# ucla-mobility/QuantV2X

Measured on AMD Instinct MI355X. Metric: frames/sec/node (N-agent int8 BEV fusion), higher is better.
Workload: dtype i8

## Files before the change

quantv2x_amd/csrc/common.h:

```cpp
#pragma once
#include <hip/hip_runtime.h>
#include <stdint.h>

#include "../../include/qv2x.h"

namespace qv2x {

int fail(int code, const char* fmt, ...);
int hip_check(hipError_t e, const char* what);

typedef int v4i __attribute__((ext_vector_type(4)));
typedef int v16i __attribute__((ext_vector_type(16)));
typedef float v4f __attribute__((ext_vector_type(4)));
typedef float v16f __attribute__((ext_vector_type(16)));

__device__ __forceinline__ float q_code(float y, float delta, float zp) {
    const float rdelta = 1.0f / delta;
    const float t = y * rdelta;
    float k = rintf(t);
    const bool doubtful = (fabsf(t - k) > 0.4997f) & (fabsf(t) < 1100.0f);
    if (__builtin_amdgcn_ballot_w64(doubtful) != 0) k = rintf(y / delta);
    float c = k + zp;
    c = fmaxf(c, 0.0f);
    return fminf(c, 255.0f);
}

__device__ __forceinline__ void q_add(float y, int e, float rdelta, float zp, float low, unsigned& c) {
    float t = __builtin_fmaf(y, rdelta, zp);
    t = fmaxf(t, low);
    c = __builtin_amdgcn_cvt_pk_u8_f32(t, e, c);
}
__device__ __forceinline__ int q_pack4(float y0, float y1, float y2, float y3, float delta, float rdelta, float zp, float lowc = 8388608.0f) {
    (void)delta;
    const float low = lowc - 8388608.0f;
    unsigned c = 0;
    q_add(y0, 0, rdelta, zp, low, c);
    q_add(y1, 1, rdelta, zp, low, c);
    q_add(y2, 2, rdelta, zp, low, c);
    q_add(y3, 3, rdelta, zp, low, c);
    return (int)(c ^ 0x80808080u);
}
__device__ __forceinline__ float q_code_mul(float y, float delta, float zp) {
    const float rdelta = 1.0f / delta;
    return fminf(fmaxf(rintf(__builtin_fmaf(y, rdelta, zp)), 0.0f), 255.0f);
}

__device__ __forceinline__ void q_sandwich_add(float y, int e, float rdelta, float za, float zb, unsigned& ca, unsigned& cb) {
    ca = __builtin_amdgcn_cvt_pk_u8_f32(__builtin_fmaf(y, rdelta, za), e, ca);
    cb = __builtin_amdgcn_cvt_pk_u8_f32(__builtin_fmaf(y, rdelta, zb), e, cb);
}
__device__ __forceinline__ int q_sandwich_finish(unsigned ca, unsigned cb, float y0, float y1, float y2, float y3, float delta, float zp, float low) {
    if ((__builtin_amdgcn_ballot_w64(ca != cb) != 0) | (low > 0.0f)) {
        const float y[4] = {y0, y1, y2, y3};
        ca = 0;
#pragma unroll
        for (int e = 0; e < 4; ++e) ca = __builtin_amdgcn_cvt_pk_u8_f32(fmaxf(rintf(y[e] / delta) + zp, low), e, ca);
    }
    return (int)(ca ^ 0x80808080u);
}
__device__ __forceinline__ int q_pack4_div(float y0, float y1, float y2, float y3, float delta, float rdelta, float zp, float lowc = 8388608.0f) {
    const float za = zp + 1.0e-4f, zb = zp - 1.0e-4f;
    unsigned ca = 0, cb = 0;
    q_sandwich_add(y0, 0, rdelta, za, zb, ca, cb);
    q_sandwich_add(y1, 1, rdelta, za, zb, ca, cb);
    q_sandwich_add(y2, 2, rdelta, za, zb, ca, cb);
    q_sandwich_add(y3, 3, rdelta, za, zb, ca, cb);
    return q_sandwich_finish(ca, cb, y0, y1, y2, y3, delta, zp, lowc - 8388608.0f);
}

__device__ __forceinline__ int mfma32_row(int r, int lane) { return (r & 3) + 8 * (r >> 2) + 4 * (lane >> 5); }

}
```

quantv2x_amd/csrc/heads_f32.hip:

```cpp
#include "fuse_att.h"

namespace qv2x {

enum { ROWS_GLOBAL = 0, ROWS_DECODE = 2, ROWS_FUSE = 3 };

#ifdef QV2X_HEADS_TRACE
__device__ long long g_heads_trace[32768 * 6];
#define HTRACE(k) do { const int hb_ = ((blockIdx.x >> 3) & 1) * (gridDim.x >> 1) + (blockIdx.x >> 4) * 8 + (blockIdx.x & 7); if (threadIdx.x == 0 && hb_ < 32768) g_heads_trace[hb_ * 6 + (k)] = __builtin_amdgcn_s_memtime(); } while (0)
#else
#define HTRACE(k) do { } while (0)
#endif

struct HeadArgs {
    const float* x; int R, hw, cout, cout_pad;
    const float* w; const float* bias; const float* da; const float* za; float* out;
};

template <int SRC, int NA = 1, bool U8 = false>
__device__ __forceinline__ void rows_heads_tile(const HeadArgs& h, const FuseArgs& fa, const int tm, float* smem, const SceneList* sl = nullptr) {
    float* rows = smem;
    HTRACE(0);
    const int lane = threadIdx.x & 63, wave = __builtin_amdgcn_readfirstlane(threadIdx.x >> 6);
    const int nct = h.cout_pad >> 5;
    const int par = lane >> 5;
// ... 152 lines not shown
            for (int hf = 0; hf < 2; ++hf)
#pragma unroll
                for (int r2 = 0; r2 < 4; ++r2) {
                    float y = c16[hf][r2];
                    if (d > 0.0f) y = U8 ? q_code(y, d, z) : (q_code(y, d, z) - z) * d;
                    tr[16 * hf + 4 * (lane >> 4) + r2][lane & 15] = y;
                }
        } else {
            const int co = ct * 32 + (lane & 31);
            const float d = h.da[co], z = h.za[co];
#pragma unroll
            for (int r2 = 0; r2 < 16; ++r2) {
                float y = acc[r2];
                if (d > 0.0f) y = U8 ? q_code(y, d, z) : (q_code(y, d, z) - z) * d;
                tr[mfma32_row(r2, lane)][lane & 31] = y;
            }
        }
        __builtin_amdgcn_s_waitcnt(0xc07f);
        __builtin_amdgcn_wave_barrier();
        const int mm = tm * 32 + (lane & 31);
        const int bi = mm / h.hw, cell = mm - bi * h.hw;
        float* ob = h.out + (size_t)bi * h.cout * h.hw + cell;
        uint8_t* ob8 = (uint8_t*)h.out + (size_t)bi * h.cout * h.hw + cell;
#pragma unroll
        for (int c = 0; c < 16; ++c) {
            const int ch = ct * 32 + par + 2 * c;
            if (ch < h.cout && mm < h.R) {
                if (U8) ob8[(size_t)ch * h.hw] = (uint8_t)tr[lane & 31][par + 2 * c];
                else ob[(size_t)ch * h.hw] = tr[lane & 31][par + 2 * c];
            }
        }
    }
    HTRACE(4);
}

template <int SRC, bool U8 = false>
__global__ __launch_bounds__(256) void rows_heads_kernel(const HeadArgs h, const FuseArgs fa) {
    __shared__ __attribute__((aligned(16))) float smem[32 * 256];
    rows_heads_tile<SRC, 1, U8>(h, fa, blockIdx.x, smem);
}

template <int NA, bool U8 = false>
__global__ __launch_bounds__(256) void fuse_heads_kernel(const HeadArgs h, const FuseArgs fa, const SceneList sl) {
    __shared__ __attribute__((aligned(16))) float smem[32 * 256];
    rows_heads_tile<ROWS_FUSE, NA, U8>(h, fa, blockIdx.x, smem, &sl);
}

__global__ __launch_bounds__(256) void rows_heads_pair_kernel(const HeadArgs h0, const HeadArgs h1, const FuseArgs fa1) {
    __shared__ __attribute__((aligned(16))) float smem[32 * 256];
    const int tile = (blockIdx.x >> 4) * 8 + (blockIdx.x & 7);
    if (((blockIdx.x >> 3) & 1) == 0) {
        if (tile * 32 < h0.R) rows_heads_tile<ROWS_GLOBAL>(h0, fa1, tile, smem);
    } else {
        if (tile * 32 < h1.R) rows_heads_tile<ROWS_DECODE>(h1, fa1, tile, smem);
    }
}

static int head_args(const char* who, int R, int hw, int cout, int cout_pad, const float* w, const float* bias, const float* da,
                     const float* za, float* out, HeadArgs& h) {
    if (!w || !bias || !da || !za || !out) return fail(QV2X_EINVAL, "%s: null pointer", who);
    if (R <= 0 || hw <= 0 || R % hw || cout <= 0 || cout > cout_pad || cout_pad % 32 || cout_pad > 96)
        return fail(QV2X_EINVAL, "%s: R=%d hw=%d cout=%d cout_pad=%d (cout_pad in {32, 64, 96})", who, R, hw, cout, cout_pad);
    if ((uintptr_t)w & 15) return fail(QV2X_EALIGN, "%s: w must be 16-byte aligned", who);
    h.x = nullptr; h.R = R; h.hw = hw; h.cout = cout; h.cout_pad = cout_pad; h.w = w; h.bias = bias; h.da = da; h.za = za; h.out = out;
    return QV2X_OK;
}

static int wire_check(const char* who, int wire, int cout, const float* da_host) {
    if (wire != QV2X_WIRE_F32 && wire != QV2X_WIRE_U8) return fail(QV2X_EINVAL, "%s: wire %d (QV2X_WIRE_F32 or QV2X_WIRE_U8)", who, wire);
    if (wire == QV2X_WIRE_U8) {
        if (!da_host) return fail(QV2X_EINVAL, "%s: the u8 wire needs da_host (the host copy of da)", who);
        for (int c = 0; c < cout; ++c)
            if (!(da_host[c] > 0.0f)) return fail(QV2X_EINVAL, "%s: the u8 wire needs an output quantizer on every channel (da[%d] = %g)", who, c, da_host[c]);
    }
    return QV2X_OK;
}

template <bool U8>
__global__ __launch_bounds__(256) void assemble_bands_kernel(const uint8_t* __restrict__ slabs, long long slab_bytes, int world, int planes, int cout,
                                                             int h, int w, const float* __restrict__ da, const float* __restrict__ za,
                                                             float* __restrict__ out) {
    const int r = blockIdx.y / planes, p = blockIdx.y - r * planes;
    const int y0 = (int)((long long)r * h / world), y1 = (int)((long long)(r + 1) * h / world);
    const int n = (y1 - y0) * w;
    if (n == 0) return;
    const size_t so = (size_t)p * n;
    const uint8_t* s8 = slabs + (size_t)r * slab_bytes + so;
    const float* s32 = (const float*)(slabs + (size_t)r * slab_bytes) + so;
    const size_t dof = (size_t)p * h * w + (size_t)y0 * w;
    float* dst = out + dof;
    float d = 1.0f, z = 0.0f;
    if (U8) { const int c = p % cout; d = da[c]; z = za[c]; }
    auto one = [&](int i) __attribute__((always_inline)) { return U8 ? ((float)s8[i] - z) * d : s32[i]; };
    int head = (int)((4 - (dof & 3)) & 3);
    if (head > n || ((so + head) & 3)) head = n;
    const int nv = (n - head) >> 2;
    const int tid = blockIdx.x * 256 + threadIdx.x, nt = gridDim.x * 256;
    for (int i = tid; i < head; i += nt) dst[i] = one(i);
    for (int v = tid; v < nv; v += nt) {
        const int i = head + 4 * v;
        float4 o;
        if (U8) {
            const unsigned cw = *(const unsigned*)(s8 + i);
            o = make_float4(((float)(cw & 0xff) - z) * d, ((float)((cw >> 8) & 0xff) - z) * d, ((float)((cw >> 16) & 0xff) - z) * d, ((float)(cw >> 24) - z) * d);
        } else {
            o = *(const float4*)(s32 + i);
        }
        *(float4*)(dst + i) = o;
    }
    for (int i = head + 4 * nv + tid; i < n; i += nt) dst[i] = one(i);
}

__global__ __launch_bounds__(256) void decode_lut_kernel(const uint8_t* __restrict__ codes, int R, int levels, int kc,
                                                         const float4* __restrict__ lut, const float4* __restrict__ bias,
                                                         float4* __restrict__ out) {
    const int lane = threadIdx.x & 63;
    int r = blockIdx.x * 4 + (threadIdx.x >> 6);
    r = __builtin_amdgcn_readfirstlane(r);
    if (r >= R) return;
    float4 v = bias[lane];
    for (int l = 0; l < levels; ++l) {
        const float4 t = lut[((size_t)l * kc + codes[(size_t)l * R + r]) * 64 + lane];
        v.x += t.x; v.y += t.y; v.z += t.z; v.w += t.w;
    }
    out[(size_t)r * 64 + lane] = v;
}

__global__ __launch_bounds__(256) void single_heads_lut_kernel(const uint8_t* __restrict__ codes, int R, int hw, int levels, int kc, int cout,
                                                               int groups, const float* __restrict__ tables, const float* __restrict__ bias,
                                                               const float* __restrict__ da, const float* __restrict__ za, float* __restrict__ out) {
    extern __shared__ __attribute__((aligned(16))) float tab[];
    const int nt = levels * kc * cout;
    for (int i = threadIdx.x; i < nt; i += blockDim.x) tab[i] = tables[i];
    for (int i = threadIdx.x; i < cout; i += blockDim.x) { tab[nt + i] = bias[i]; tab[nt + cout + i] = da[i]; tab[nt + 2 * cout + i] = za[i]; }
    __syncthreads();
    const int lane = threadIdx.x & 63, wv = threadIdx.x >> 6;
    for (int g = 0; g < groups; ++g) {
        const int m = (blockIdx.x * groups + g) * 64 + lane;
        if (m >= R) break;
        const int agent = m / hw, cell = m - agent * hw;
        const float* row[4];
        for (int l = 0; l < levels; ++l) row[l] = tab + ((size_t)l * kc + codes[(size_t)l * R + m]) * cout;
        float* ob = out + (size_t)agent * cout * hw + cell;
        for (int c = wv; c < cout; c += 4) {
            float y = tab[nt + c];
            for (int l = 0; l < levels; ++l) y += row[l][c];
            const float d = tab[nt + cout + c], z = tab[nt + 2 * cout + c];
            if (d > 0.0f) y = (q_code(y, d, z) - z) * d;
            ob[(size_t)c * hw] = y;
        }
    }
}

__global__ __launch_bounds__(1024, 1) void table_heads_kernel(const uint8_t* __restrict__ codes, int R, int hw, int levels, int kc, int CT, int ST, int c0, int c1,
                                                             const float* __restrict__ tables, const float* __restrict__ bias, const float* __restrict__ da,
                                                             const float* __restrict__ za, float* __restrict__ out0, float* __restrict__ out1) {
    extern __shared__ __attribute__((aligned(16))) float tab[];
    const int CT4 = (CT + 3) & ~3, rows = levels * kc;
    float* cst = tab + (size_t)rows * ST;
    for (int i = threadIdx.x; i < rows * (ST / 4); i += blockDim.x) {
        const int row = i / (ST / 4), q = i - row * (ST / 4);
        v4f v = {0.f, 0.f, 0.f, 0.f};
#pragma unroll
        for (int e = 0; e < 4; ++e)
            if (4 * q + e < CT) v[e] = tables[(size_t)row * CT + 4 * q + e];
        *(v4f*)(tab + (size_t)row * ST + 4 * q) = v;
    }
    for (int i = threadIdx.x; i < CT4; i += blockDim.x) {
        cst[i] = i < CT ? bias[i] : 0.f; cst[CT4 + i] = i < CT ? da[i] : -1.f; cst[2 * CT4 + i] = i < CT ? za[i] : 0.f;
    }
    __syncthreads();
    const int lane = threadIdx.x & 63, wave = threadIdx.x >> 6, nw = blockDim.x >> 6;
    const int runs = (R + 63) / 64;
    for (int run = blockIdx.x * nw + wave; run < runs; run += gridDim.x * nw) {
        const int m = run * 64 + lane;
        const int mc = m < R ? m : R - 1;
        const int agent = mc / hw, cell = mc - agent * hw;
        const float* rp[4];
#pragma unroll
        for (int l = 0; l < 4; ++l) rp[l] = tab + (size_t)(l < levels ? l * kc + codes[(size_t)l * R + mc] : 0) * ST;
        float* o0 = out0 ? out0 + (size_t)agent * c0 * hw + cell : nullptr;
        float* o1 = out1 ? out1 + (size_t)agent * c1 * hw + cell : nullptr;
        for (int g = 0; g < CT4 / 4; ++g) {
            v4f y = *(const v4f*)(cst + 4 * g);
            const v4f d4 = *(const v4f*)(cst + CT4 + 4 * g), z4 = *(const v4f*)(cst + 2 * CT4 + 4 * g);
#pragma unroll
            for (int l = 0; l < 4; ++l)
                if (l < levels) { const v4f t = *(const v4f*)(rp[l] + 4 * g); y[0] += t[0]; y[1] += t[1]; y[2] += t[2]; y[3] += t[3]; }
#pragma unroll
            for (int e = 0; e < 4; ++e) {
                const int c = 4 * g + e;
                float v = y[e];
                if (d4[e] > 0.0f) v = (q_code(v, d4[e], z4[e]) - z4[e]) * d4[e];
                if (m < R && c < CT) {
                    if (c < c0) { if (o0) o0[(size_t)c * hw] = v; }
                    else if (o1) o1[(size_t)(c - c0) * hw] = v;
                }
            }
        }
    }
}

__global__ __launch_bounds__(256) void dequant_i8_kernel(const int8_t* __restrict__ in, int n, int h, int w, int c, int ax, float delta,
                                                         float* __restrict__ out) {
    const size_t total = (size_t)n * h * w * (c / 4);
    for (size_t i = (size_t)blockIdx.x * blockDim.x + threadIdx.x; i < total; i += (size_t)gridDim.x * blockDim.x) {
        const int c4 = (int)(i % (c / 4));
        const size_t pix = i / (c / 4);
        const int x = (int)(pix % w), y = (int)((pix / w) % h), img = (int)(pix / ((size_t)w * h));
        const char4 v = *(const char4*)(in + (((size_t)img * (h + 2) + y + 1) * (w + 2) + x + 1) * c + c4 * 4);
        *(float4*)(out + pix * c + c4 * 4) = make_float4((float)((int)v.x + ax) * delta, (float)((int)v.y + ax) * delta,
                                                         (float)((int)v.z + ax) * delta, (float)((int)v.w + ax) * delta);
    }
}

}

extern "C" int qv2x_dequant_i8_f32(const int8_t* in, int n, int h, int w, int c, int zp, float delta, float* out, void* stream) {
    using namespace qv2x;
    if (!in || !out) return fail(QV2X_EINVAL, "qv2x_dequant_i8_f32: null pointer");
    if (n <= 0 || h <= 0 || w <= 0 || c <= 0 || c % 4) return fail(QV2X_EINVAL, "qv2x_dequant_i8_f32: bad shape (c %% 4 == 0)");
    const size_t total = (size_t)n * h * w * (c / 4);
    const int blocks = (int)((total + 255) / 256 < 4096 ? (total + 255) / 256 : 4096);
    dequant_i8_kernel<<<blocks, 256, 0, (hipStream_t)stream>>>(in, n, h, w, c, 128 - zp, delta, out);
    return hip_check(hipGetLastError(), "qv2x_dequant_i8_f32 launch");
}

extern "C" int qv2x_heads_f32(const float* x, int R, int hw, int cout, int cout_pad, const float* w, const float* bias,
                              const float* da, const float* za, float* out, void* stream) {
    using namespace qv2x;
    HeadArgs h;
    if (!x) return fail(QV2X_EINVAL, "qv2x_heads_f32: null pointer");
    if (int rc = head_args("qv2x_heads_f32", R, hw, cout, cout_pad, w, bias, da, za, out, h)) return rc;
    if ((uintptr_t)x & 15) return fail(QV2X_EALIGN, "qv2x_heads_f32: x must be 16-byte aligned");
    h.x = x;
    rows_heads_kernel<ROWS_GLOBAL><<<(R + 31) / 32, 256, 0, (hipStream_t)stream>>>(h, FuseArgs{});
    return hip_check(hipGetLastError(), "qv2x_heads_f32 launch");
}

namespace qv2x {
static int fuse_heads_launch(const char* who, const qv2x_fuse_desc* d, int n_scenes, const int64_t* scene_offset, const int32_t* scene_agents,
                             const uint8_t* codes, const float* lut, const float* lut_bias, const float* feats, const double* pairwise,
                             const long long* range, int cout, int cout_pad, const float* w, const float* bias, const float* da, const float* za,
                             bool u8, void* out, float* fused_tap, void* stream) {
    if (!scene_offset || !scene_agents || !d) return fail(QV2X_EINVAL, "%s: null pointer", who);
    if (n_scenes < 1 || n_scenes > MAX_SCENES) return fail(QV2X_EINVAL, "%s: 1..%d scenes, got %d", who, MAX_SCENES, n_scenes);
    SceneList sl{};
    int most = 1;
    for (int s = 0; s < n_scenes; ++s) {
        if (scene_offset[s] < 0 || (feats && scene_offset[s] % 4) || scene_agents[s] < 1 || scene_agents[s] > MAXA || scene_agents[s] > d->max_cav || d->ego >= scene_agents[s])
            return fail(QV2X_EINVAL, "%s: scene %d: offset %lld, agents %d (1..%d, <= max_cav, > ego)", who, s, (long long)scene_offset[s], scene_agents[s], MAXA);
        sl.off[s] = scene_offset[s]; sl.agents[s] = scene_agents[s];
        most = scene_agents[s] > most ? scene_agents[s] : most;
    }
    qv2x_fuse_desc d1 = *d;
    d1.agents = most;
    FuseArgs a;
    if (int rc = fuse_args_from_desc(&d1, codes, lut, lut_bias, feats, pairwise, who, a)) return rc;
    if (range) {
        if (int rc = fuse_band_range(who, range[0], range[1], a)) return rc;
        if (!out) return fail(QV2X_EINVAL, "%s: null pointer", who);
        if (a.n_cells == 0) return QV2X_OK;
    }
    a.fused = (float4*)fused_tap;
    HeadArgs h;
    if (int rc = head_args(who, n_scenes * a.n_cells, a.n_cells, cout, cout_pad, w, bias, da, za, (float*)out, h)) return rc;
    const dim3 grid((h.R + 31) / 32);
    hipStream_t st = (hipStream_t)stream;
    if (u8) {
        switch (fuse_bound(most)) {
            case 1: fuse_heads_kernel<1, true><<<grid, 256, 0, st>>>(h, a, sl); break;
            case 2: fuse_heads_kernel<2, true><<<grid, 256, 0, st>>>(h, a, sl); break;
            case 4: fuse_heads_kernel<4, true><<<grid, 256, 0, st>>>(h, a, sl); break;
            default: fuse_heads_kernel<MAXA, true><<<grid, 256, 0, st>>>(h, a, sl); break;
        }
        return hip_check(hipGetLastError(), who);
    }
    switch (fuse_bound(most)) {
        case 1: fuse_heads_kernel<1><<<grid, 256, 0, st>>>(h, a, sl); break;
        case 2: fuse_heads_kernel<2><<<grid, 256, 0, st>>>(h, a, sl); break;
        case 4: fuse_heads_kernel<4><<<grid, 256, 0, st>>>(h, a, sl); break;
        default: fuse_heads_kernel<MAXA><<<grid, 256, 0, st>>>(h, a, sl); break;
    }
    return hip_check(hipGetLastError(), who);
}
}

extern "C" int qv2x_fuse_heads_batch_f32(const qv2x_fuse_desc* d, int n_scenes, const int64_t* scene_offset, const int32_t* scene_agents,
                                         const uint8_t* codes, const float* lut, const float* lut_bias, const float* feats, const double* pairwise,
                                         int cout, int cout_pad, const float* w, const float* bias, const float* da, const float* za,
                                         float* out, float* fused_tap, void* stream) {
    return qv2x::fuse_heads_launch("qv2x_fuse_heads_batch_f32", d, n_scenes, scene_offset, scene_agents, codes, lut, lut_bias, feats, pairwise, nullptr,
                                   cout, cout_pad, w, bias, da, za, false, out, fused_tap, stream);
}

extern "C" int qv2x_fuse_heads_band(const qv2x_fuse_desc* d, int n_scenes, const int64_t* scene_offset, const int32_t* scene_agents,
                                    const uint8_t* codes, const float* lut, const float* lut_bias, const float* feats, const double* pairwise,
                                    int64_t cell0, int64_t n_cells, int cout, int cout_pad, const float* w, const float* bias, const float* da,
                                    const float* za, int wire, const float* da_host, void* out, float* fused_tap, void* stream) {
    using namespace qv2x;
    if (int rc = wire_check("qv2x_fuse_heads_band", wire, cout, da_host)) return rc;
    const long long range[2] = {(long long)cell0, (long long)n_cells};
    return fuse_heads_launch("qv2x_fuse_heads_band", d, n_scenes, scene_offset, scene_agents, codes, lut, lut_bias, feats, pairwise, range,
                             cout, cout_pad, w, bias, da, za, wire == QV2X_WIRE_U8, out, fused_tap, stream);
}

extern "C" int qv2x_heads_band(const float* x, int n_scenes, int64_t n_cells, int cout, int cout_pad, const float* w, const float* bias,
                               const float* da, const float* za, int wire, const float* da_host, void* out, void* stream) {
    using namespace qv2x;
    const char* who = "qv2x_heads_band";
    if (int rc = wire_check(who, wire, cout, da_host)) return rc;
    if (!x || !out) return fail(QV2X_EINVAL, "%s: null pointer", who);
    if (n_scenes < 1 || n_cells < 0 || n_cells * n_scenes > 0x7fffffffLL) return fail(QV2X_EINVAL, "%s: %d scenes of %lld cells", who, n_scenes, (long long)n_cells);
    if (n_cells == 0) return QV2X_OK;
    HeadArgs h;
    if (int rc = head_args(who, (int)(n_scenes * n_cells), (int)n_cells, cout, cout_pad, w, bias, da, za, (float*)out, h)) return rc;
    if ((uintptr_t)x & 15) return fail(QV2X_EALIGN, "%s: x must be 16-byte aligned", who);
    h.x = x;
    if (wire == QV2X_WIRE_U8) rows_heads_kernel<ROWS_GLOBAL, true><<<(h.R + 31) / 32, 256, 0, (hipStream_t)stream>>>(h, FuseArgs{});
    else rows_heads_kernel<ROWS_GLOBAL><<<(h.R + 31) / 32, 256, 0, (hipStream_t)stream>>>(h, FuseArgs{});
    return hip_check(hipGetLastError(), who);
}

extern "C" int qv2x_assemble_bands(const uint8_t* slabs, int world, int64_t slab_bytes, int frames, int cout, int h, int w, int wire,
                                   const float* da, const float* za, float* out, void* stream) {
    using namespace qv2x;
    const char* who = "qv2x_assemble_bands";
    if (!slabs || !out) return fail(QV2X_EINVAL, "%s: null pointer", who);
    if (wire != QV2X_WIRE_F32 && wire != QV2X_WIRE_U8) return fail(QV2X_EINVAL, "%s: wire %d (QV2X_WIRE_F32 or QV2X_WIRE_U8)", who, wire);
    if (wire == QV2X_WIRE_U8 && (!da || !za)) return fail(QV2X_EINVAL, "%s: the u8 wire needs da and za", who);
    if (world < 1 || frames < 1 || cout < 1 || h < 1 || w < 1 || (long long)h * w > 0x7fffffffLL || (long long)world * frames * cout > 65535)
        return fail(QV2X_EINVAL, "%s: world=%d frames=%d cout=%d h=%d w=%d (world * frames * cout <= 65535)", who, world, frames, cout, h, w);
    const long long cap = (long long)((h + world - 1) / world) * w, need = (long long)frames * cout * cap * (wire == QV2X_WIRE_U8 ? 1 : 4);
    if (slab_bytes < need || slab_bytes % 16) return fail(QV2X_EINVAL, "%s: slab_bytes %lld (>= %lld, a multiple of 16)", who, (long long)slab_bytes, need);
    if (((uintptr_t)slabs & 15) || ((uintptr_t)out & 15)) return fail(QV2X_EALIGN, "%s: slabs and out must be 16-byte aligned", who);
    const int planes = frames * cout;
    const long long quads = (cap + 3) / 4;
    const dim3 grid((unsigned)((quads + 255) / 256 < 64 ? (quads + 255) / 256 : 64), (unsigned)(world * planes));
    if (wire == QV2X_WIRE_U8) assemble_bands_kernel<true><<<grid, 256, 0, (hipStream_t)stream>>>(slabs, slab_bytes, world, planes, cout, h, w, da, za, out);
    else assemble_bands_kernel<false><<<grid, 256, 0, (hipStream_t)stream>>>(slabs, slab_bytes, world, planes, cout, h, w, da, za, out);
    return hip_check(hipGetLastError(), who);
}

extern "C" int qv2x_decode_heads_f32(const uint8_t* codes, int R, int hw, int levels, int kc, const float* lut, const float* lut_bias,
                                     int cout, int cout_pad, const float* w, const float* bias, const float* da, const float* za,
                                     float* out, void* stream) {
    using namespace qv2x;
    if (!codes || !lut || !lut_bias) return fail(QV2X_EINVAL, "qv2x_decode_heads_f32: null pointer");
    if (levels < 1 || levels > 16 || kc < 1 || kc > 256) return fail(QV2X_EINVAL, "qv2x_decode_heads_f32: bad sizes (1..16 code planes = levels * seg_num, dict_size <= 256)");
    HeadArgs h;
    if (int rc = head_args("qv2x_decode_heads_f32", R, hw, cout, cout_pad, w, bias, da, za, out, h)) return rc;
    FuseArgs fa{};
    fa.codes = codes; fa.lut = (const float4*)lut; fa.lut_bias = (const float4*)lut_bias; fa.feats = nullptr;
    fa.levels = levels; fa.kc = kc; fa.hw = hw;
    fa.code_agent_stride = hw; fa.code_level_stride = R;
    rows_heads_kernel<ROWS_DECODE><<<(R + 31) / 32, 256, 0, (hipStream_t)stream>>>(h, fa);
    return hip_check(hipGetLastError(), "qv2x_decode_heads_f32 launch");
}

extern "C" int qv2x_single_heads_lut_f32(const uint8_t* codes, int R, int hw, int levels, int kc, int cout, const float* tables,
                                         const float* bias, const float* da, const float* za, float* out, void* stream) {
    using namespace qv2x;
    if (!codes || !tables || !bias || !da || !za || !out) return fail(QV2X_EINVAL, "qv2x_single_heads_lut_f32: null pointer");
    if (R <= 0 || hw <= 0 || R % hw || levels < 1 || levels > 4 || kc < 1 || kc > 256 || cout < 1 || cout > 96)
        return fail(QV2X_EINVAL, "qv2x_single_heads_lut_f32: R=%d hw=%d levels=%d kc=%d cout=%d", R, hw, levels, kc, cout);
    const size_t lds = ((size_t)levels * kc * cout + 3 * cout) * sizeof(float);
    if (lds > 64 * 1024) return fail(QV2X_EINVAL, "qv2x_single_heads_lut_f32: tables of %zu bytes do not fit the 64 KB of LDS this kernel takes", lds);
    const int runs = (R + 63) / 64;
    const int groups = runs <= 1024 ? 1 : (runs + 1023) / 1024;
    single_heads_lut_kernel<<<(runs + groups - 1) / groups, 256, lds, (hipStream_t)stream>>>(codes, R, hw, levels, kc, cout, groups, tables, bias, da, za, out);
    return hip_check(hipGetLastError(), "qv2x_single_heads_lut_f32 launch");
}

namespace qv2x {
__global__ __launch_bounds__(1024, 1) void table_heads4_kernel(const uint8_t* __restrict__ codes, int R, int hw, int levels, int kc, int CT, int ST, int c0, int c1,
                                                              const float* __restrict__ tables, const float* __restrict__ bias, const float* __restrict__ da,
                                                              const float* __restrict__ za, float* __restrict__ out0, float* __restrict__ out1) {
    extern __shared__ __attribute__((aligned(16))) float tab[];
    const int CT4 = (CT + 3) & ~3, rows = levels * kc;
    float* cst = tab + (size_t)rows * ST;
    for (int i = threadIdx.x; i < rows * (ST / 4); i += blockDim.x) {
        const int row = i / (ST / 4), q = i - row * (ST / 4);
        v4f v = {0.f, 0.f, 0.f, 0.f};
#pragma unroll
        for (int e = 0; e < 4; ++e)
            if (4 * q + e < CT) v[e] = tables[(size_t)row * CT + 4 * q + e];
        *(v4f*)(tab + (size_t)row * ST + 4 * q) = v;
    }
    for (int i = threadIdx.x; i < CT4; i += blockDim.x) {
        cst[i] = i < CT ? bias[i] : 0.f; cst[CT4 + i] = i < CT ? da[i] : -1.f; cst[2 * CT4 + i] = i < CT ? za[i] : 0.f;
        cst[3 * CT4 + i] = i < CT && da[i] > 0.0f ? 1.0f / da[i] : 0.f;
    }
    __syncthreads();
    const int lane = threadIdx.x & 63, wave = threadIdx.x >> 6, nw = blockDim.x >> 6;
    const int runs = (R + 255) / 256;
    for (int run = blockIdx.x * nw + wave; run < runs; run += gridDim.x * nw) {
        const int m = run * 256 + 4 * lane;
        const int mc = m < R ? m : R - 4;
        const int agent = mc / hw, cell = mc - agent * hw;
        const float* rp[4][4];
#pragma unroll
        for (int l = 0; l < 4; ++l) {
            const unsigned cw = l < levels ? *(const unsigned*)(codes + (size_t)l * R + mc) : 0u;
#pragma unroll
            for (int j = 0; j < 4; ++j) rp[l][j] = tab + (size_t)(l < levels ? l * kc + ((cw >> (8 * j)) & 0xff) : 0) * ST;
        }
        float* o0 = out0 ? out0 + (size_t)agent * c0 * hw + cell : nullptr;
        float* o1 = out1 ? out1 + (size_t)agent * c1 * hw + cell : nullptr;
        for (int g = 0; g < CT4 / 4; ++g) {
            const v4f b4 = *(const v4f*)(cst + 4 * g), d4 = *(const v4f*)(cst + CT4 + 4 * g), z4 = *(const v4f*)(cst + 2 * CT4 + 4 * g);
            const v4f r4 = *(const v4f*)(cst + 3 * CT4 + 4 * g);
            v4f y[4];
#pragma unroll
            for (int j = 0; j < 4; ++j) {
                y[j] = b4;
#pragma unroll
                for (int l = 0; l < 4; ++l)
                    if (l < levels) { const v4f t = *(const v4f*)(rp[l][j] + 4 * g); y[j][0] += t[0]; y[j][1] += t[1]; y[j][2] += t[2]; y[j][3] += t[3]; }
            }
#pragma unroll
            for (int e = 0; e < 4; ++e) {
                const int c = 4 * g + e;
                v4f v = {y[0][e], y[1][e], y[2][e], y[3][e]};
                if (d4[e] > 0.0f) {
                    const unsigned cw = (unsigned)q_pack4_div(v[0], v[1], v[2], v[3], d4[e], r4[e], z4[e]) ^ 0x80808080u;
                    v[0] = ((float)(cw & 0xff) - z4[e]) * d4[e];
                    v[1] = ((float)((cw >> 8) & 0xff) - z4[e]) * d4[e];
                    v[2] = ((float)((cw >> 16) & 0xff) - z4[e]) * d4[e];
                    v[3] = ((float)(cw >> 24) - z4[e]) * d4[e];
                }
                if (m < R && c < CT) {
                    if (c < c0) { if (o0) *(v4f*)(o0 + (size_t)c * hw) = v; }
                    else if (o1) *(v4f*)(o1 + (size_t)(c - c0) * hw) = v;
                }
            }
        }
    }
}

constexpr int TG_CELLS = 32, TG_PITCH = 33;
__global__ __launch_bounds__(256) void table_heads_global_kernel(const uint8_t* __restrict__ codes, int R, int hw, int planes, int kc, int CT, int c0, int c1,
                                                                 const float* __restrict__ tables, const float* __restrict__ bias, const float* __restrict__ da,
                                                                 const float* __restrict__ za, float* __restrict__ out0, float* __restrict__ out1) {
    extern __shared__ __attribute__((aligned(16))) float tg[];
    const int lane = threadIdx.x & 63, wave = threadIdx.x >> 6, half = lane >> 5, l31 = lane & 31;
    float* tr = tg + (size_t)wave * CT * TG_PITCH;
    const int run = __builtin_amdgcn_readfirstlane((int)(blockIdx.x * 4 + wave));
    const int m0 = run * TG_CELLS;
    if (m0 >= R) return;
    const int mc = m0 + l31 < R ? m0 + l31 : R - 1;
    int code[16];
#pragma unroll
    for (int p = 0; p < 16; ++p) code[p] = p < planes ? (int)codes[(size_t)p * R + mc] : 0;
    const int ch = 4 * l31;
    const bool chan = ch < CT;
    v4f b4 = {0.f, 0.f, 0.f, 0.f}, d4 = {-1.f, -1.f, -1.f, -1.f}, z4 = {0.f, 0.f, 0.f, 0.f};
    if (chan) { b4 = *(const v4f*)(bias + ch); d4 = *(const v4f*)(da + ch); z4 = *(const v4f*)(za + ch); }
    const float* tcol = tables + (chan ? ch : 0);
#pragma unroll 2
    for (int it = 0; it < TG_CELLS / 2; ++it) {
        const int cell = 2 * it + half;
        v4f t[16];
#pragma unroll
        for (int p = 0; p < 16; ++p) {
            if (p < planes) {
                const int lo = __builtin_amdgcn_readlane(code[p], 2 * it), hi = __builtin_amdgcn_readlane(code[p], 2 * it + 1);
                t[p] = *(const v4f*)(tcol + (size_t)(p * kc + (half ? hi : lo)) * CT);
            }
        }
        v4f y = b4;
#pragma unroll
        for (int p = 0; p < 16; ++p)
            if (p < planes) y += t[p];
        if (chan) {
#pragma unroll
            for (int e = 0; e < 4; ++e) {
                float v = y[e];
                if (d4[e] > 0.0f) v = (q_code(v, d4[e], z4[e]) - z4[e]) * d4[e];
                tr[(ch + e) * TG_PITCH + cell] = v;
            }
        }
    }
    __builtin_amdgcn_s_waitcnt(0xc07f);
    __builtin_amdgcn_wave_barrier();
    const int mm = m0 + l31;
    if (mm < R) {
        const int agent = mm / hw, cl = mm - agent * hw;
        float* o0 = out0 ? out0 + (size_t)agent * c0 * hw + cl : nullptr;
        float* o1 = out1 ? out1 + (size_t)agent * c1 * hw + cl : nullptr;
        for (int c = half; c < CT; c += 2) {
            const float v = tr[c * TG_PITCH + l31];
            if (c < c0) o0[(size_t)c * hw] = v; else o1[(size_t)(c - c0) * hw] = v;
        }
    }
}
}

extern "C" int qv2x_table_heads_f32(const uint8_t* codes, int R, int hw, int levels, int kc, int c0, int c1, const float* tables,
                                    const float* bias, const float* da, const float* za, float* out0, float* out1, void* stream) {
    using namespace qv2x;
    const char* who = "qv2x_table_heads_f32";
    if (!codes || !tables || !bias || !da || !za || (!out0 && !out1)) return fail(QV2X_EINVAL, "%s: null pointer", who);
    const int CT = c0 + c1;
    if (R <= 0 || hw <= 0 || R % hw || levels < 1 || levels > 16 || kc < 1 || kc > 256 || c0 < 0 || c1 < 0 || CT < 1 || (c0 > 0) != (out0 != nullptr) || (c1 > 0) != (out1 != nullptr))
        return fail(QV2X_EINVAL, "%s: R=%d hw=%d levels=%d kc=%d c0=%d c1=%d (1..16 planes; an output per non-empty channel set)", who, R, hw, levels, kc, c0, c1);
    const int CT4 = (CT + 3) & ~3;
    const int ST = (CT4 / 4) % 2 ? CT4 : CT4 + 4;
    const size_t lds = ((size_t)levels * kc * ST + 4 * CT4) * sizeof(float);
    if (levels > 4 || lds > 160 * 1024) {
        if (CT % 4 || CT > 128 || ((uintptr_t)tables & 15) || ((uintptr_t)bias & 15) || ((uintptr_t)da & 15) || ((uintptr_t)za & 15))
            return fail(QV2X_EINVAL, "%s: tables past the 160 KB of LDS need c0 + c1 %% 4 == 0, <= 128, and 16-byte aligned arrays", who);
        const size_t tl = (size_t)4 * CT * TG_PITCH * sizeof(float);
        if (int rc = hip_check(hipFuncSetAttribute((const void*)table_heads_global_kernel, hipFuncAttributeMaxDynamicSharedMemorySize, (int)tl), who)) return rc;
        const int runs = (R + TG_CELLS - 1) / TG_CELLS;
        table_heads_global_kernel<<<(runs + 3) / 4, 256, tl, (hipStream_t)stream>>>(codes, R, hw, levels, kc, CT, c0, c1, tables, bias, da, za, out0, out1);
        return hip_check(hipGetLastError(), "qv2x_table_heads_f32 launch");
    }
    if (int rc = hip_check(hipFuncSetAttribute((const void*)table_heads_kernel, hipFuncAttributeMaxDynamicSharedMemorySize, (int)lds), who)) return rc;
    int dev = 0, cus = 256, v = 0;
    if (hipGetDevice(&dev) == hipSuccess && hipDeviceGetAttribute(&v, hipDeviceAttributeMultiprocessorCount, dev) == hipSuccess && v > 0) cus = v;
    int cells_per_lane = 4;
#ifdef QV2X_DEV_KNOBS
    static const int cells_env = getenv("QV2X_TABLE_HEADS_CELLS") ? atoi(getenv("QV2X_TABLE_HEADS_CELLS")) : 4;
    cells_per_lane = cells_env;
#endif
    if (cells_per_lane == 4 && hw % 4 == 0 && (R + 255) / 256 >= 16 * cus && !((uintptr_t)codes & 3) && !((uintptr_t)out0 & 15) && !((uintptr_t)out1 & 15)) {
        if (int rc = hip_check(hipFuncSetAttribute((const void*)table_heads4_kernel, hipFuncAttributeMaxDynamicSharedMemorySize, (int)lds), who)) return rc;
        table_heads4_kernel<<<cus, 1024, lds, (hipStream_t)stream>>>(codes, R, hw, levels, kc, CT, ST, c0, c1, tables, bias, da, za, out0, out1);
        return hip_check(hipGetLastError(), "qv2x_table_heads_f32 launch");
    }
    const int runs = (R + 63) / 64;
    const int nwav = runs >= 16 * cus ? 16 : 8, want = (runs + nwav - 1) / nwav;
    table_heads_kernel<<<want < cus ? want : cus, nwav * 64, lds, (hipStream_t)stream>>>(codes, R, hw, levels, kc, CT, ST, c0, c1, tables, bias, da, za, out0, out1);
    return hip_check(hipGetLastError(), "qv2x_table_heads_f32 launch");
}

extern "C" int qv2x_decode_lut_f32(const uint8_t* codes, int R, int levels, int kc, const float* lut, const float* lut_bias,
                                   float* out, void* stream) {
    using namespace qv2x;
    if (!codes || !lut || !lut_bias || !out) return fail(QV2X_EINVAL, "qv2x_decode_lut_f32: null pointer");
    if (R <= 0 || levels < 1 || levels > 16 || kc < 1 || kc > 256) return fail(QV2X_EINVAL, "qv2x_decode_lut_f32: bad sizes (1..16 code planes = levels * seg_num, dict_size <= 256)");
    decode_lut_kernel<<<(R + 3) / 4, 256, 0, (hipStream_t)stream>>>(codes, R, levels, kc, (const float4*)lut, (const float4*)lut_bias, (float4*)out);
    return hip_check(hipGetLastError(), "qv2x_decode_lut_f32 launch");
}

#ifdef QV2X_HEADS_TRACE
extern "C" __attribute__((visibility("default"))) int qv2x_debug_heads_trace(long long* host_out, int nblocks) {
    using namespace qv2x;
    return (int)hipMemcpyFromSymbol(host_out, HIP_SYMBOL(g_heads_trace), (size_t)nblocks * 6 * sizeof(long long));
}
#endif

extern "C" int qv2x_heads_pair_f32(const float* x, int R, int hw, int cout, int cout_pad, const float* w, const float* bias,
                                   const float* da, const float* za, float* out,
                                   const uint8_t* codes, int R1, int levels, int kc, const float* lut, const float* lut_bias,
                                   int cout1, int cout_pad1, const float* w1, const float* bias1, const float* da1,
                                   const float* za1, float* out1, void* stream) {
    using namespace qv2x;
    HeadArgs h0, h1;
    if (!x || !codes || !lut || !lut_bias) return fail(QV2X_EINVAL, "qv2x_heads_pair_f32: null pointer");
    if (int rc = head_args("qv2x_heads_pair_f32", R, hw, cout, cout_pad, w, bias, da, za, out, h0)) return rc;
    if (int rc = head_args("qv2x_heads_pair_f32", R1, hw, cout1, cout_pad1, w1, bias1, da1, za1, out1, h1)) return rc;
    if ((uintptr_t)x & 15) return fail(QV2X_EALIGN, "qv2x_heads_pair_f32: x must be 16-byte aligned");
    if (levels < 1 || levels > 16 || kc < 1 || kc > 256) return fail(QV2X_EINVAL, "qv2x_heads_pair_f32: bad sizes (1..16 code planes = levels * seg_num, dict_size <= 256)");
    h0.x = x;
    FuseArgs fa{};
    fa.codes = codes; fa.lut = (const float4*)lut; fa.lut_bias = (const float4*)lut_bias; fa.feats = nullptr;
    fa.levels = levels; fa.kc = kc; fa.hw = hw;
    fa.code_agent_stride = hw; fa.code_level_stride = R1;
    const int tiles = ((R > R1 ? R : R1) + 31) / 32;
    rows_heads_pair_kernel<<<dim3(16 * ((tiles + 7) / 8)), 256, 0, (hipStream_t)stream>>>(h0, h1, fa);
    return hip_check(hipGetLastError(), "qv2x_heads_pair_f32 launch");
}
```

Baseline: 6749.

## Specialize table-heads kernels on level count with fused bias and uniform quant fast path

Result: faster. 6869, median of 5 (+1.8%).

```diff
diff --git a/quantv2x_amd/csrc/common.h b/quantv2x_amd/csrc/common.h
--- a/quantv2x_amd/csrc/common.h
+++ b/quantv2x_amd/csrc/common.h
@@ -68,6 +68,25 @@
     return q_sandwich_finish(ca, cb, y0, y1, y2, y3, delta, zp, lowc - 8388608.0f);
 }
 
+__device__ __forceinline__ unsigned q_exact_add(float y, int e, float delta, float zp, unsigned c) {
+    return __builtin_amdgcn_cvt_pk_u8_f32(fmaxf(rintf(y / delta) + zp, 0.0f), e, c);
+}
+template <int E>
+__device__ __forceinline__ float q_byte_f32(unsigned c) { return (float)((c >> (8 * E)) & 0xffu); }
+
+inline int device_cu_count() {
+    static int cached[64];
+    int dev = 0;
+    if (hipGetDevice(&dev) != hipSuccess || dev < 0 || dev >= 64) return 256;
+    int n = __atomic_load_n(&cached[dev], __ATOMIC_RELAXED);
+    if (n == 0) {
+        int v = 0;
+        n = hipDeviceGetAttribute(&v, hipDeviceAttributeMultiprocessorCount, dev) == hipSuccess && v > 0 ? v : 256;
+        __atomic_store_n(&cached[dev], n, __ATOMIC_RELAXED);
+    }
+    return n;
+}
+
 __device__ __forceinline__ int mfma32_row(int r, int lane) { return (r & 3) + 8 * (r >> 2) + 4 * (lane >> 5); }
 
 }
diff --git a/quantv2x_amd/csrc/heads_f32.hip b/quantv2x_amd/csrc/heads_f32.hip
--- a/quantv2x_amd/csrc/heads_f32.hip
+++ b/quantv2x_amd/csrc/heads_f32.hip
@@ -328,52 +328,136 @@
     }
 }
 
-__global__ __launch_bounds__(1024, 1) void table_heads_kernel(const uint8_t* __restrict__ codes, int R, int hw, int levels, int kc, int CT, int ST, int c0, int c1,
+template <bool VEC>
+__device__ __forceinline__ void table_heads_copy_rows(float* tab, int rows, int kc, int CT, int SQ, const float* __restrict__ tables, const float* __restrict__ bias) {
+    const int total = rows * SQ;
+    constexpr int U = 8;
+    for (int i0 = threadIdx.x; i0 < total; i0 += U * blockDim.x) {
+        v4f t[U], b[U];
+#pragma unroll
+        for (int u = 0; u < U; ++u) {
+            const int i = i0 + u * blockDim.x, ic = i < total ? i : total - 1;
+            const int row = ic / SQ, q = ic - row * SQ;
+            if (VEC) {
+                const int qc = 4 * q < CT ? q : 0;
+                t[u] = *(const v4f*)(tables + (size_t)row * CT + 4 * qc);
+                b[u] = *(const v4f*)(bias + 4 * qc);
+            } else {
+#pragma unroll
+                for (int e = 0; e < 4; ++e) {
+                    const int cc = 4 * q + e < CT ? 4 * q + e : CT - 1;
+                    t[u][e] = tables[(size_t)row * CT + cc]; b[u][e] = bias[cc];
+                }
+            }
+        }
+#pragma unroll
+        for (int u = 0; u < U; ++u) {
+            const int i = i0 + u * blockDim.x, ic = i < total ? i : total - 1;
+            const int row = ic / SQ, q = ic - row * SQ;
+            v4f v;
+#pragma unroll
+            for (int e = 0; e < 4; ++e) {
+                float x = t[u][e];
+                if (row < kc) x = b[u][e] + x;
+                v[e] = 4 * q + e < CT ? x : 0.f;
+            }
+            if (i < total) *(v4f*)(tab + 4 * (size_t)i) = v;
+        }
+    }
+}
+__device__ __forceinline__ const float* table_heads_copy_in(float* tab, int planes, int kc, int CT, int ST, const float* __restrict__ tables,
+                                                            const float* __restrict__ bias, const float* __restrict__ da, const float* __restrict__ za) {
+    const int CT4 = (CT + 3) & ~3, rows = planes * kc;
+    float* cst = tab + (size_t)rows * ST;
+    if (CT % 4 == 0 && !(((uintptr_t)tables | (uintptr_t)bias) & 15)) table_heads_copy_rows<true>(tab, rows, kc, CT, ST / 4, tables, bias);
+    else table_heads_copy_rows<false>(tab, rows, kc, CT, ST / 4, tables, bias);
+    for (int i = threadIdx.x; i < CT4; i += blockDim.x) {
+        const int ic = i < CT ? i : CT - 1;
+        const float d = da[ic], z = za[ic];
+        const bool quant = i < CT && d > 0.0f;
+        cst[i] = quant ? d : -1.f; cst[CT4 + i] = i < CT ? z : 0.f;
+        cst[2 * CT4 + i] = quant ? 1.0f / d : 0.f; cst[3 * CT4 + i] = i < CT ? z + 1.0e-4f : 0.f;
+    }
+    __syncthreads();
+    return cst;
+}
+
+__device__ __forceinline__ bool table_heads_all_quantized(const v4f d4) {
+    const float m = fminf(fminf(fminf(d4[0], d4[1]), d4[2]), d4[3]);
+    return __builtin_amdgcn_readfirstlane(__float_as_int(m)) > 0;
+}
+
+__device__ __forceinline__ void table_heads_store(float* p, float v) {
+#ifdef QV2X_TABLE_HEADS_NO_STORE
+    asm volatile("" :: "v"(p), "v"(v));
+#else
+    *p = v;
+#endif
+}
+__device__ __forceinline__ void table_heads_store(float* p, v4f v) {
+#ifdef QV2X_TABLE_HEADS_NO_STORE
+    asm volatile("" :: "v"(p), "v"(v));
+#else
+    *(v4f*)p = v;
+#endif
+}
+
+template <int LV, bool WHOLE>
+__device__ __forceinline__ void table_heads1_group(const float* cst, int CT4, const float* (&rp)[LV], int g, int CT, int c0, int hw,
+                                                   float* o0, float* o1, float* of) {
+    v4f y = *(const v4f*)(rp[0] + 4 * g);
+#pragma unroll
+    for (int l = 1; l < LV; ++l) y += *(const v4f*)(rp[l] + 4 * g);
+    const v4f d4 = *(const v4f*)(cst + 4 * g), z4 = *(const v4f*)(cst + CT4 + 4 * g);
+    v4f v = y;
+    if (table_heads_all_quantized(d4)) {
+        const v4f r4 = *(const v4f*)(cst + 2 * CT4 + 4 * g), za4 = *(const v4f*)(cst + 3 * CT4 + 4 * g);
+        unsigned ca = 0, cb = 0;
+#pragma unroll
+        for (int e = 0; e < 4; ++e) q_sandwich_add(y[e], e, r4[e], za4[e], z4[e] - 1.0e-4f, ca, cb);
+        if (__builtin_amdgcn_ballot_w64(ca != cb) != 0) {
+            ca = 0;
+#pragma unroll
+            for (int e = 0; e < 4; ++e) ca = q_exact_add(y[e], e, d4[e], z4[e], ca);
+        }
+        v[0] = (q_byte_f32<0>(ca) - z4[0]) * d4[0]; v[1] = (q_byte_f32<1>(ca) - z4[1]) * d4[1];
+        v[2] = (q_byte_f32<2>(ca) - z4[2]) * d4[2]; v[3] = (q_byte_f32<3>(ca) - z4[3]) * d4[3];
+    } else {
+#pragma unroll
+        for (int e = 0; e < 4; ++e)
+            if (d4[e] > 0.0f) v[e] = (q_code(y[e], d4[e], z4[e]) - z4[e]) * d4[e];
+    }
+#pragma unroll
+    for (int e = 0; e < 4; ++e) {
+        const int c = 4 * g + e;
+        if (WHOLE) table_heads_store(of + (size_t)e * hw, v[e]);
+        else if (c < CT) table_heads_store(c < c0 ? o0 + (size_t)c * hw : o1 + (size_t)(c - c0) * hw, v[e]);
+    }
+}
+
+template <int LV>
+__global__ __launch_bounds__(1024, 1) void table_heads_kernel(const uint8_t* __restrict__ codes, int R, int hw, int kc, int CT, int ST, int c0, int c1,
                                                              const float* __restrict__ tables, const float* __restrict__ bias, const float* __restrict__ da,
                                                              const float* __restrict__ za, float* __restrict__ out0, float* __restrict__ out1) {
     extern __shared__ __attribute__((aligned(16))) float tab[];
-    const int CT4 = (CT + 3) & ~3, rows = levels * kc;
-    float* cst = tab + (size_t)rows * ST;
-    for (int i = threadIdx.x; i < rows * (ST / 4); i += blockDim.x) {
-        const int row = i / (ST / 4), q = i - row * (ST / 4);
-        v4f v = {0.f, 0.f, 0.f, 0.f};
-#pragma unroll
-        for (int e = 0; e < 4; ++e)
-            if (4 * q + e < CT) v[e] = tables[(size_t)row * CT + 4 * q + e];
-        *(v4f*)(tab + (size_t)row * ST + 4 * q) = v;
-    }
-    for (int i = threadIdx.x; i < CT4; i += blockDim.x) {
-        cst[i] = i < CT ? bias[i] : 0.f; cst[CT4 + i] = i < CT ? da[i] : -1.f; cst[2 * CT4 + i] = i < CT ? za[i] : 0.f;
-    }
-    __syncthreads();
+    const int CT4 = (CT + 3) & ~3;
+    const float* cst = table_heads_copy_in(tab, LV, kc, CT, ST, tables, bias, da, za);
     const int lane = threadIdx.x & 63, wave = threadIdx.x >> 6, nw = blockDim.x >> 6;
     const int runs = (R + 63) / 64;
+    const int ga = c0 >> 2, gb = (c0 + 3) >> 2, gc = CT >> 2;
     for (int run = blockIdx.x * nw + wave; run < runs; run += gridDim.x * nw) {
         const int m = run * 64 + lane;
-        const int mc = m < R ? m : R - 1;
-        const int agent = mc / hw, cell = mc - agent * hw;
-        const float* rp[4];
-#pragma unroll
-        for (int l = 0; l < 4; ++l) rp[l] = tab + (size_t)(l < levels ? l * kc + codes[(size_t)l * R + mc] : 0) * ST;
-        float* o0 = out0 ? out0 + (size_t)agent * c0 * hw + cell : nullptr;
-        float* o1 = out1 ? out1 + (size_t)agent * c1 * hw + cell : nullptr;
-        for (int g = 0; g < CT4 / 4; ++g) {
-            v4f y = *(const v4f*)(cst + 4 * g);
-            const v4f d4 = *(const v4f*)(cst + CT4 + 4 * g), z4 = *(const v4f*)(cst + 2 * CT4 + 4 * g);
-#pragma unroll
-            for (int l = 0; l < 4; ++l)
-                if (l < levels) { const v4f t = *(const v4f*)(rp[l] + 4 * g); y[0] += t[0]; y[1] += t[1]; y[2] += t[2]; y[3] += t[3]; }
-#pragma unroll
-            for (int e = 0; e < 4; ++e) {
-                const int c = 4 * g + e;
-                float v = y[e];
-                if (d4[e] > 0.0f) v = (q_code(v, d4[e], z4[e]) - z4[e]) * d4[e];
-                if (m < R && c < CT) {
-                    if (c < c0) { if (o0) o0[(size_t)c * hw] = v; }
-                    else if (o1) o1[(size_t)(c - c0) * hw] = v;
-                }
-            }
-        }
+        if (m >= R) continue;
+        const int agent = m / hw, cell = m - agent * hw;
+        const float* rp[LV];
+#pragma unroll
+        for (int l = 0; l < LV; ++l) rp[l] = tab + (size_t)(l * kc + codes[(size_t)l * R + m]) * ST;
+        float* o0 = out0 + (size_t)agent * c0 * hw + cell;
+        float* o1 = out1 + (size_t)agent * c1 * hw + cell;
+        for (int g = 0; g < ga; ++g) table_heads1_group<LV, true>(cst, CT4, rp, g, CT, c0, hw, o0, o1, o0 + (size_t)(4 * g) * hw);
+        if (c0 & 3) table_heads1_group<LV, false>(cst, CT4, rp, ga, CT, c0, hw, o0, o1, nullptr);
+        for (int g = gb; g < gc; ++g) table_heads1_group<LV, true>(cst, CT4, rp, g, CT, c0, hw, o0, o1, o1 + (size_t)(4 * g - c0) * hw);
+        if ((CT & 3) && !((c0 & 3) && gc == ga)) table_heads1_group<LV, false>(cst, CT4, rp, gc, CT, c0, hw, o0, o1, nullptr);
     }
 }
 
@@ -549,68 +633,89 @@
 }
 
 namespace qv2x {
-__global__ __launch_bounds__(1024, 1) void table_heads4_kernel(const uint8_t* __restrict__ codes, int R, int hw, int levels, int kc, int CT, int ST, int c0, int c1,
+template <int LV, bool WHOLE>
+__device__ __forceinline__ void table_heads4_group(const float* cst, int CT4, const float* (&rp)[LV][4], int g, int CT, int c0, int hw,
+                                                   float* o0, float* o1, float* of) {
+    v4f y[4];
+#pragma unroll
+    for (int j = 0; j < 4; ++j) y[j] = *(const v4f*)(rp[0][j] + 4 * g);
+#pragma unroll
+    for (int l = 1; l < LV; ++l)
+#pragma unroll
+        for (int j = 0; j < 4; ++j) y[j] += *(const v4f*)(rp[l][j] + 4 * g);
+    const v4f d4 = *(const v4f*)(cst + 4 * g), z4 = *(const v4f*)(cst + CT4 + 4 * g);
+    v4f v[4];
+    if (table_heads_all_quantized(d4)) {
+        const v4f r4 = *(const v4f*)(cst + 2 * CT4 + 4 * g), za4 = *(const v4f*)(cst + 3 * CT4 + 4 * g);
+        unsigned ca[4], cb[4], differ = 0;
+#pragma unroll
+        for (int e = 0; e < 4; ++e) {
+            const float zb = z4[e] - 1.0e-4f;
+            ca[e] = 0; cb[e] = 0;
+#pragma unroll
+            for (int j = 0; j < 4; ++j) q_sandwich_add(y[j][e], j, r4[e], za4[e], zb, ca[e], cb[e]);
+            differ |= ca[e] ^ cb[e];
+        }
+        if (__builtin_amdgcn_ballot_w64(differ != 0) != 0) {
+#pragma unroll
+            for (int e = 0; e < 4; ++e) {
+                ca[e] = 0;
+#pragma unroll
+                for (int j = 0; j < 4; ++j) ca[e] = q_exact_add(y[j][e], j, d4[e], z4[e], ca[e]);
+            }
+        }
+#pragma unroll
+        for (int e = 0; e < 4; ++e)
+            v[e] = v4f{(q_byte_f32<0>(ca[e]) - z4[e]) * d4[e], (q_byte_f32<1>(ca[e]) - z4[e]) * d4[e],
+                       (q_byte_f32<2>(ca[e]) - z4[e]) * d4[e], (q_byte_f32<3>(ca[e]) - z4[e]) * d4[e]};
+    } else {
+#pragma unroll
+        for (int e = 0; e < 4; ++e) {
+            v[e] = v4f{y[0][e], y[1][e], y[2][e], y[3][e]};
+            if (d4[e] > 0.0f) {
+                const unsigned cw = (unsigned)q_pack4_div(v[e][0], v[e][1], v[e][2], v[e][3], d4[e], 1.0f / d4[e], z4[e]) ^ 0x80808080u;
+                v[e] = v4f{(q_byte_f32<0>(cw) - z4[e]) * d4[e], (q_byte_f32<1>(cw) - z4[e]) * d4[e],
+                           (q_byte_f32<2>(cw) - z4[e]) * d4[e], (q_byte_f32<3>(cw) - z4[e]) * d4[e]};
+            }
+        }
+    }
+#pragma unroll
+    for (int e = 0; e < 4; ++e) {
+        const int c = 4 * g + e;
+        if (WHOLE) table_heads_store(of + (size_t)e * hw, v[e]);
+        else if (c < CT) table_heads_store(c < c0 ? o0 + (size_t)c * hw : o1 + (size_t)(c - c0) * hw, v[e]);
+    }
+}
+
+template <int LV>
+__global__ __launch_bounds__(1024, 1) void table_heads4_kernel(const uint8_t* __restrict__ codes, int R, int hw, int kc, int CT, int ST, int c0, int c1,
                                                               const float* __restrict__ tables, const float* __restrict__ bias, const float* __restrict__ da,
                                                               const float* __restrict__ za, float* __restrict__ out0, float* __restrict__ out1) {
     extern __shared__ __attribute__((aligned(16))) float tab[];
-    const int CT4 = (CT + 3) & ~3, rows = levels * kc;
-    float* cst = tab + (size_t)rows * ST;
-    for (int i = threadIdx.x; i < rows * (ST / 4); i += blockDim.x) {
-        const int row = i / (ST / 4), q = i - row * (ST / 4);
-        v4f v = {0.f, 0.f, 0.f, 0.f};
-#pragma unroll
-        for (int e = 0; e < 4; ++e)
-            if (4 * q + e < CT) v[e] = tables[(size_t)row * CT + 4 * q + e];
-        *(v4f*)(tab + (size_t)row * ST + 4 * q) = v;
-    }
-    for (int i = threadIdx.x; i < CT4; i += blockDim.x) {
-        cst[i] = i < CT ? bias[i] : 0.f; cst[CT4 + i] = i < CT ? da[i] : -1.f; cst[2 * CT4 + i] = i < CT ? za[i] : 0.f;
-        cst[3 * CT4 + i] = i < CT && da[i] > 0.0f ? 1.0f / da[i] : 0.f;
-    }
-    __syncthreads();
+    const int CT4 = (CT + 3) & ~3;
+    const float* cst = table_heads_copy_in(tab, LV, kc, CT, ST, tables, bias, da, za);
     const int lane = threadIdx.x & 63, wave = threadIdx.x >> 6, nw = blockDim.x >> 6;
     const int runs = (R + 255) / 256;
-    for (int run = blockIdx.x * nw + wave; run < runs; run += gridDim.x * nw) {
+    const int ga = c0 >> 2, gb = (c0 + 3) >> 2, gc = CT >> 2;
+    for (int run = wave * gridDim.x + blockIdx.x; run < runs; run += gridDim.x * nw) {
         const int m = run * 256 + 4 * lane;
-        const int mc = m < R ? m : R - 4;
-        const int agent = mc / hw, cell = mc - agent * hw;
-        const float* rp[4][4];
-#pragma unroll
-        for (int l = 0; l < 4; ++l) {
-            const unsigned cw = l < levels ? *(const unsigned*)(codes + (size_t)l * R + mc) : 0u;
-#pragma unroll
-            for (int j = 0; j < 4; ++j) rp[l][j] = tab + (size_t)(l < levels ? l * kc + ((cw >> (8 * j)) & 0xff) : 0) * ST;
-        }
-        float* o0 = out0 ? out0 + (size_t)agent * c0 * hw + cell : nullptr;
-        float* o1 = out1 ? out1 + (size_t)agent * c1 * hw + cell : nullptr;
-        for (int g = 0; g < CT4 / 4; ++g) {
-            const v4f b4 = *(const v4f*)(cst + 4 * g), d4 = *(const v4f*)(cst + CT4 + 4 * g), z4 = *(const v4f*)(cst + 2 * CT4 + 4 * g);
-            const v4f r4 = *(const v4f*)(cst + 3 * CT4 + 4 * g);
-            v4f y[4];
-#pragma unroll
-            for (int j = 0; j < 4; ++j) {
-                y[j] = b4;
-#pragma unroll
-                for (int l = 0; l < 4; ++l)
-                    if (l < levels) { const v4f t = *(const v4f*)(rp[l][j] + 4 * g); y[j][0] += t[0]; y[j][1] += t[1]; y[j][2] += t[2]; y[j][3] += t[3]; }
-            }
-#pragma unroll
-            for (int e = 0; e < 4; ++e) {
-                const int c = 4 * g + e;
-                v4f v = {y[0][e], y[1][e], y[2][e], y[3][e]};
-                if (d4[e] > 0.0f) {
-                    const unsigned cw = (unsigned)q_pack4_div(v[0], v[1], v[2], v[3], d4[e], r4[e], z4[e]) ^ 0x80808080u;
-                    v[0] = ((float)(cw & 0xff) - z4[e]) * d4[e];
-                    v[1] = ((float)((cw >> 8) & 0xff) - z4[e]) * d4[e];
-                    v[2] = ((float)((cw >> 16) & 0xff) - z4[e]) * d4[e];
-                    v[3] = ((float)(cw >> 24) - z4[e]) * d4[e];
-                }
-                if (m < R && c < CT) {
-                    if (c < c0) { if (o0) *(v4f*)(o0 + (size_t)c * hw) = v; }
-                    else if (o1) *(v4f*)(o1 + (size_t)(c - c0) * hw) = v;
-                }
-            }
-        }
+        if (m >= R) continue;
+        const int agent = m / hw, cell = m - agent * hw;
+        const float* rp[LV][4];
+#pragma unroll
+        for (int l = 0; l < LV; ++l) {
+            const unsigned cw = *(const unsigned*)(codes + (size_t)l * R + m);
+#pragma unroll
+            for (int j = 0; j < 4; ++j) rp[l][j] = tab + (size_t)(l * kc + ((cw >> (8 * j)) & 0xff)) * ST;
+        }
+        float* o0 = out0 + (size_t)agent * c0 * hw + cell;
+        float* o1 = out1 + (size_t)agent * c1 * hw + cell;
+#pragma unroll 2
+        for (int g = 0; g < ga; ++g) table_heads4_group<LV, true>(cst, CT4, rp, g, CT, c0, hw, o0, o1, o0 + (size_t)(4 * g) * hw);
+        if (c0 & 3) table_heads4_group<LV, false>(cst, CT4, rp, ga, CT, c0, hw, o0, o1, nullptr);
+#pragma unroll 2
+        for (int g = gb; g < gc; ++g) table_heads4_group<LV, true>(cst, CT4, rp, g, CT, c0, hw, o0, o1, o1 + (size_t)(4 * g - c0) * hw);
+        if ((CT & 3) && !((c0 & 3) && gc == ga)) table_heads4_group<LV, false>(cst, CT4, rp, gc, CT, c0, hw, o0, o1, nullptr);
     }
 }
 
@@ -669,6 +774,18 @@
             if (c < c0) o0[(size_t)c * hw] = v; else o1[(size_t)(c - c0) * hw] = v;
         }
     }
+}
+
+struct TableHeadsLaunch { bool four; int grid, threads; size_t lds; hipStream_t stream; };
+template <int LV>
+static int table_heads_lds(const TableHeadsLaunch& tl, const uint8_t* codes, int R, int hw, int kc, int CT, int ST, int c0, int c1, const float* tables,
+                           const float* bias, const float* da, const float* za, float* out0, float* out1) {
+    const char* who = "qv2x_table_heads_f32";
+    const void* fn = tl.four ? (const void*)table_heads4_kernel<LV> : (const void*)table_heads_kernel<LV>;
+    if (int rc = hip_check(hipFuncSetAttribute(fn, hipFuncAttributeMaxDynamicSharedMemorySize, (int)tl.lds), who)) return rc;
+    if (tl.four) table_heads4_kernel<LV><<<tl.grid, tl.threads, tl.lds, tl.stream>>>(codes, R, hw, kc, CT, ST, c0, c1, tables, bias, da, za, out0, out1);
+    else table_heads_kernel<LV><<<tl.grid, tl.threads, tl.lds, tl.stream>>>(codes, R, hw, kc, CT, ST, c0, c1, tables, bias, da, za, out0, out1);
+    return hip_check(hipGetLastError(), "qv2x_table_heads_f32 launch");
 }
 }
 
@@ -692,23 +809,22 @@
         table_heads_global_kernel<<<(runs + 3) / 4, 256, tl, (hipStream_t)stream>>>(codes, R, hw, levels, kc, CT, c0, c1, tables, bias, da, za, out0, out1);
         return hip_check(hipGetLastError(), "qv2x_table_heads_f32 launch");
     }
-    if (int rc = hip_check(hipFuncSetAttribute((const void*)table_heads_kernel, hipFuncAttributeMaxDynamicSharedMemorySize, (int)lds), who)) return rc;
-    int dev = 0, cus = 256, v = 0;
-    if (hipGetDevice(&dev) == hipSuccess && hipDeviceGetAttribute(&v, hipDeviceAttributeMultiprocessorCount, dev) == hipSuccess && v > 0) cus = v;
+    const int cus = device_cu_count();
     int cells_per_lane = 4;
 #ifdef QV2X_DEV_KNOBS
     static const int cells_env = getenv("QV2X_TABLE_HEADS_CELLS") ? atoi(getenv("QV2X_TABLE_HEADS_CELLS")) : 4;
     cells_per_lane = cells_env;
 #endif
-    if (cells_per_lane == 4 && hw % 4 == 0 && (R + 255) / 256 >= 16 * cus && !((uintptr_t)codes & 3) && !((uintptr_t)out0 & 15) && !((uintptr_t)out1 & 15)) {
-        if (int rc = hip_check(hipFuncSetAttribute((const void*)table_heads4_kernel, hipFuncAttributeMaxDynamicSharedMemorySize, (int)lds), who)) return rc;
-        table_heads4_kernel<<<cus, 1024, lds, (hipStream_t)stream>>>(codes, R, hw, levels, kc, CT, ST, c0, c1, tables, bias, da, za, out0, out1);
-        return hip_check(hipGetLastError(), "qv2x_table_heads_f32 launch");
-    }
+    const bool four = cells_per_lane == 4 && hw % 4 == 0 && (R + 255) / 256 >= 16 * cus && !((uintptr_t)codes & 3) && !((uintptr_t)out0 & 15) && !((uintptr_t)out1 & 15);
     const int runs = (R + 63) / 64;
-    const int nwav = runs >= 16 * cus ? 16 : 8, want = (runs + nwav - 1) / nwav;
-    table_heads_kernel<<<want < cus ? want : cus, nwav * 64, lds, (hipStream_t)stream>>>(codes, R, hw, levels, kc, CT, ST, c0, c1, tables, bias, da, za, out0, out1);
-    return hip_check(hipGetLastError(), "qv2x_table_heads_f32 launch");
+    const int nwav = four || runs >= 16 * cus ? 16 : 8, want = (runs + nwav - 1) / nwav;
+    const TableHeadsLaunch tl{four, four || want > cus ? cus : want, nwav * 64, lds, (hipStream_t)stream};
+    switch (levels) {
+        case 1: return table_heads_lds<1>(tl, codes, R, hw, kc, CT, ST, c0, c1, tables, bias, da, za, out0, out1);
+        case 2: return table_heads_lds<2>(tl, codes, R, hw, kc, CT, ST, c0, c1, tables, bias, da, za, out0, out1);
+        case 3: return table_heads_lds<3>(tl, codes, R, hw, kc, CT, ST, c0, c1, tables, bias, da, za, out0, out1);
+        default: return table_heads_lds<4>(tl, codes, R, hw, kc, CT, ST, c0, c1, tables, bias, da, za, out0, out1);
+    }
 }
 
 extern "C" int qv2x_decode_lut_f32(const uint8_t* codes, int R, int levels, int kc, const float* lut, const float* lut_bias,
```
